# UWRobotLearning/WheeledLab

Measured on AMD Instinct MI355X. Metric: env steps/sec (whole node), drift task @ 4096 envs/GPU, higher is better.
Workload: dtype f32; 1 GPU; drift task, 4096 envs/GPU, flat terrain, fused step kernel, synthetic actions in HBM; envs_per_gpu=4096, total_envs=4096, parallelism=env-shard x1

## Files before the change

wheeledlab_amd/csrc/wl_drift.hip:

```cpp
#include "wl_drift_env.h"

namespace {

constexpr int kHotArgBytes = 56;

template <int LANES, class Ground, bool UNROLL = true, int DRIVE = -1, int QB = kBlock, bool STREAM = false>
__global__ void __launch_bounds__(kBlock, LANES == 4 ? WL_MIN_WAVES : (UNROLL ? WL_LANE_WAVES : WL_LOWREG_WAVES)) drift_step_kernel(float* __restrict__ state, int32_t* __restrict__ episode_len,
                                                            const float2* __restrict__ actions, const int stride,
                                                            const int n_envs, const int env_offset, const uint64_t seed,
                                                            const uint64_t step, const WlDriftParams p_arg,
                                                            const VehDerived vd_arg, const WlEnvBuffers b_arg,
                                                            const float* __restrict__ noise, const WlStepOut out,
                                                            const Ground ground, const MetricSlots slots) {
    constexpr int kEnvs = QB / LANES;
    WlDriftParams p = p_arg;
    VehDerived vd = vd_arg;
    WlEnvBuffers b = b_arg;
    b.state = state;
    b.episode_len = episode_len;
    b.stride = stride;
    b.n_envs = n_envs;
    b.env_offset = env_offset;
    __shared__ float tile[LANES == 1 ? kEnvs * kObsPad : 1];
    __shared__ float wave_metrics[LANES == 1 ? (QB / 64) * WL_M_COUNT : 1];
// ... 12 lines not shown
        float dr_mass, dr_mu_s, dr_mu_d, dr_damp;
        dr_mass = S.ld(WL_S_MASS, e), dr_mu_s = S.ld(WL_S_MU_S, e), dr_mu_d = S.ld(WL_S_MU_D, e), dr_damp = S.ld(WL_S_DAMP, e);
        load_rows<LANES>(S, b, p, e, wid, r);
        const uint32_t gid = (uint32_t)(b.env_offset + e);
        float* tile_w = tile + (LANES == 1 ? wave * 64 * kObsPad : 0);
        if constexpr (LANES == 4) {
            uint32_t kw[(sizeof(WlDriftParams) + sizeof(VehDerived)) / 4];
            kernarg_vector_words(kHotArgBytes, kw);
            int go = 1;
            asm volatile("" : "+s"(go) : : "memory");
            if (go) {
                StepDraws pre = draw_step_raw(gid, step, seed, wid);
                kernarg_words_landed(kw);
                __builtin_memcpy(&p, kw, sizeof(WlDriftParams));
                __builtin_memcpy(&vd, kw + sizeof(WlDriftParams) / 4, sizeof(VehDerived));
                keep_scalar_fields(p, p_arg);
                vd.n_sub = uniform_i32(vd.n_sub);
                ref_pose_request(pre, b.ref_poses, p.num_ref_points);
                env_const_rows(ec, p.vehicle, vd, dr_mass, dr_mu_s, dr_mu_d, dr_damp);
                drift_env_step<LANES>(p, b, vd, ground, S, ec, r, a, noise, out, e, wid, lead, gid, seed, step, tile_w, ms, nullptr, &pre);
            }
        } else {
            env_const_rows(ec, p.vehicle, vd, dr_mass, dr_mu_s, dr_mu_d, dr_damp);
            drift_env_step<LANES, UNROLL, DRIVE>(p, b, vd, ground, S, ec, r, a, noise, out, e, wid, lead, gid, seed, step, tile_w, ms);
        }
        store_rows<LANES>(S, b, p, e, wid, lead, r);
    }
    if (b.metrics_slots > 1) clear_metric_slot(b, slots.next);
    if constexpr (LANES == 1) {
        const int wave_env0 = blockIdx.x * kEnvs + wave * 64;
        if (wave_env0 < b.n_envs) flush_obs_wave<kStreaming>(tile + wave * 64 * kObsPad, out.obs, wave_env0, b.n_envs);
        ms.close();
    }
}

template <class Ground, int QB = kBlock >
__global__ void __launch_bounds__(kBlock) drift_rollout_kernel(const WlDriftParams p_arg, const WlEnvBuffers b,
                                                               const float2* __restrict__ actions, const WlStepOut out,
                                                               const int64_t obs_step_stride, const int64_t vec_step_stride,
                                                               const int n_steps, const uint64_t seed, const uint64_t step0,
                                                               const Ground ground, const VehDerived vd_arg, const MetricSlots slots) {
    constexpr int LANES = 4, kEnvs = QB / LANES;
    WlDriftParams p = p_arg;
    VehDerived vd = vd_arg;
    pin_params_vgpr(p, vd);
    const int wid = threadIdx.x & 3;
    const bool lead = wid == 0;
    const int e = blockIdx.x * kEnvs + threadIdx.x / LANES;
    if (b.metrics_slots > 1) clear_metric_slot(b, slots.next);
    if (e >= b.n_envs) return;
    const MetricSink<LANES> ms{nullptr, metric_shard(b, slots.cur)};
    const Rows S = make_rows(b.state, b.stride);
    EnvConst ec;
    DriftRows r;
    load_env_const(S, p.vehicle, vd, e, ec);
    load_rows<LANES>(S, b, p, e, wid, r);
    const uint32_t gid = (uint32_t)(b.env_offset + e);
    float2 a_next = n_steps > 0 ? actions[e] : make_float2(0.f, 0.f);
    for (int k = 0; k < n_steps; ++k) {
        WlStepOut o = out;
        o.obs += k * obs_step_stride;
        o.reward += k * vec_step_stride;
        o.terminated += k * vec_step_stride;
        o.truncated += k * vec_step_stride;
        if (o.dones) o.dones += k * vec_step_stride;
        const float2 a = a_next;
        if (k + 1 < n_steps) a_next = actions[(int64_t)(k + 1) * b.n_envs + e];
        const StepDraws pre = draw_step(p, b.ref_poses, gid, step0 + (uint64_t)k, seed, wid);
        drift_env_step<LANES>(p, b, vd, ground, S, ec, r, a, nullptr, o, e, wid, lead, gid, seed, step0 + (uint64_t)k, nullptr, ms,
                              nullptr, &pre);
    }
    store_rows<LANES>(S, b, p, e, wid, lead, r);
}

constexpr int kSplitEnvs = 16;
constexpr int kSplitBlock = 128;
constexpr int kSnapVec = 6, kDrawVec = 3;

WL_DEV void snap_publish(float4* slot, int q, const DriftSnap& s) {
    float4* w = slot + q * kSnapVec;
    w[0] = make_float4(s.pos.x, s.pos.y, s.pos.z, s.q.w);
    w[1] = make_float4(s.q.x, s.q.y, s.q.z, s.v.x);
    w[2] = make_float4(s.v.y, s.v.z, s.wb.x, s.wb.y);
    w[3] = make_float4(s.wb.z, s.wwz, s.th, s.a0);
    w[4] = make_float4(s.a1, __int_as_float(s.ep_len), __int_as_float(s.flags), s.dvx);
    w[5] = make_float4(s.dvy, s.dwz_hf, s.dwz_lf, 0.f);
}
WL_DEV DriftSnap snap_read(const float4* slot, int q) {
    const float4* w = slot + q * kSnapVec;
    const float4 w0 = w[0], w1 = w[1], w2 = w[2], w3 = w[3], w4 = w[4], w5 = w[5];
    DriftSnap s;
    s.pos = v3(w0.x, w0.y, w0.z), s.q = Quat{w0.w, w1.x, w1.y, w1.z}, s.v = v3(w1.w, w2.x, w2.y), s.wb = v3(w2.z, w2.w, w3.x);
    s.wwz = w3.y, s.th = w3.z, s.a0 = w3.w, s.a1 = w4.x, s.ep_len = __float_as_int(w4.y), s.flags = __float_as_int(w4.z);
    s.dvx = w4.w, s.dvy = w5.x, s.dwz_hf = w5.y, s.dwz_lf = w5.z;
    return s;
}
WL_DEV void draws_publish(float4* slot, int q, const DriftEventDraws& d) {
    float4* w = slot + q * kDrawVec;
    w[0] = make_float4(d.rx, d.ry, d.rqw, d.rqz);
    w[1] = make_float4(d.rt_hf, d.rt_lf, d.lf_kick, d.lf_timer);
    w[2] = make_float4(d.hf.x, d.hf.y, d.hf.z, d.hf.w);
}
WL_DEV DriftEventDraws draws_read(const float4* slot, int q) {
    const float4* w = slot + q * kDrawVec;
    const float4 w0 = w[0], w1 = w[1], w2 = w[2];
    DriftEventDraws d;
    d.rx = w0.x, d.ry = w0.y, d.rqw = w0.z, d.rqz = w0.w, d.rt_hf = w1.x, d.rt_lf = w1.y, d.lf_kick = w1.z, d.lf_timer = w1.w;
    d.hf = F4{w2.x, w2.y, w2.z, w2.w};
    return d;
}

template <class Ground>
__global__ void __launch_bounds__(kSplitBlock) drift_rollout_split_kernel(const WlDriftParams p_arg, const WlEnvBuffers b,
                                                                          const float2* __restrict__ actions, const WlStepOut out,
                                                                          const int64_t obs_step_stride, const int64_t vec_step_stride,
                                                                          const int n_steps, const uint64_t seed, const uint64_t step0,
                                                                          const Ground ground, const VehDerived vd_arg, const MetricSlots slots) {
    __shared__ float4 snap[2][kSplitEnvs * kSnapVec];
    __shared__ float4 drw[2][kSplitEnvs * kDrawVec];
    WlDriftParams p = p_arg;
    VehDerived vd = vd_arg;
    const int role = __builtin_amdgcn_readfirstlane((int)threadIdx.x >> 6);
    const int wid = threadIdx.x & 3, q = (threadIdx.x & 63) >> 2;
    const int e_quad = blockIdx.x * kSplitEnvs + q;
    if (b.metrics_slots > 1) clear_metric_slot(b, slots.next);
    if (blockIdx.x * kSplitEnvs >= b.n_envs) return;
    const bool live = e_quad < b.n_envs;
    const int e = live ? e_quad : b.n_envs - 1;
    const bool lead = wid == 0;
    const Rows S = make_rows(b.state, b.stride);
    const uint32_t gid = (uint32_t)(b.env_offset + e);
    if (role == 0) {
        pin_state_params_vgpr(p, vd);
        EnvConst ec;
        DriftRows r;
        load_env_const(S, p.vehicle, vd, e, ec);
        load_rows<4>(S, b, p, e, wid, r);
        float2 a_next = n_steps > 0 ? actions[e] : make_float2(0.f, 0.f);
        __syncthreads();
        for (int k = 0; k < n_steps; ++k) {
            const float2 a = a_next;
            if (k + 1 < n_steps) a_next = actions[(int64_t)(k + 1) * b.n_envs + e];
            const DriftEventDraws dr = draws_read(drw[k & 1], q);
            const DriftSnap sn = drift_state_half(p, vd, ground, ec, r, a, wid, dr);
            if (lead) snap_publish(snap[k & 1], q, sn);
            __syncthreads();
        }
        if (live) {
            WlDriftParams ps = p;
            ps.log_episode_sums = 0;
            store_rows<4>(S, b, ps, e, wid, lead, r);
        }
    } else {
        pin_output_params_vgpr(p);
        const MetricSink<4> ms{nullptr, metric_shard(b, slots.cur)};
        float epsum[WL_DR_NTERMS];
#pragma unroll
        for (int i = 0; i < WL_DR_NTERMS; ++i) epsum[i] = S.ld(WL_S_EPSUM0 + i, e);
        StepDraws d = draw_step(p, b.ref_poses, gid, step0, seed, wid);
        ResetDraw rd = quad_reset_draw(p, d);
        const DriftEventDraws ev0 = event_draws(rd, d);
        if (lead) draws_publish(drw[0], q, ev0);
        __syncthreads();
        for (int k = 0; k < n_steps; ++k) {
            WlStepOut o = out;
            o.obs += k * obs_step_stride;
            o.reward += k * vec_step_stride;
            o.terminated += k * vec_step_stride;
            o.truncated += k * vec_step_stride;
            if (o.dones) o.dones += k * vec_step_stride;
            const StepDraws dn = draw_step(p, b.ref_poses, gid, step0 + (uint64_t)(k + 1), seed, wid);
            const ResetDraw rdn = quad_reset_draw(p, dn);
            const DriftEventDraws evn = event_draws(rdn, dn);
            if (lead) draws_publish(drw[(k + 1) & 1], q, evn);
            __syncthreads();
            const DriftSnap sn = snap_read(snap[k & 1], q);
            drift_output_half(p, o, sn, rd, d.z, epsum, e, wid, live, ms);
            d = dn;
            rd = rdn;
        }
        if (live && lead && p.log_episode_sums) {
#pragma unroll
            for (int i = 0; i < WL_DR_NTERMS; ++i) S.st(WL_S_EPSUM0 + i, e, epsum[i]);
        }
    }
}

__global__ void __launch_bounds__(kBlock) drift_mdp_kernel(const WlDriftParams p, int n, int64_t stride,
                                                           const float* __restrict__ pos, const float* __restrict__ quat,
                                                           const float* __restrict__ vb_, const float* __restrict__ wb_,
                                                           const float* __restrict__ ww_, const float* __restrict__ steer,
                                                           const float* __restrict__ act, const uint8_t* __restrict__ timed_out,
                                                           float* __restrict__ terms, float* __restrict__ reward,
                                                           uint8_t* __restrict__ terminated, float* __restrict__ obs) {
    __shared__ float tile[kBlock * kObsPad];
    const int e = blockIdx.x * kBlock + threadIdx.x;
    if (e < n) {
        const V3 P = v3(pos[e], pos[stride + e], pos[2 * stride + e]);
        const Quat q{quat[e], quat[stride + e], quat[2 * stride + e], quat[3 * stride + e]};
        const V3 vb = v3(vb_[e], vb_[stride + e], vb_[2 * stride + e]);
        const V3 wb = v3(wb_[e], wb_[stride + e], wb_[2 * stride + e]);
        const float wwz = ww_[2 * stride + e];
        const float sm = 0.5f * (steer[e] + steer[stride + e]);
        const bool to = timed_out ? timed_out[e] != 0 : false;
        const bool term = cart_off_track(P.x, P.y, p.straight, p.r_in, p.r_out);
        const DriftTerms tm = drift_terms(p, P, vb, wb, wwz, sm, term, to, atan2_fast(vb.y, vb.x));
        const float step_dt = p.sim_dt * (float)p.decimation;
        float r = 0.f;
#pragma unroll
        for (int i = 0; i < WL_DR_NTERMS; ++i) {
            terms[i * stride + e] = tm.t[i];
            if (p.weight[i] != 0.f) r += tm.t[i] * p.weight[i] * step_dt;
        }
        reward[e] = r;
        terminated[e] = term ? 1 : 0;
        Noise12 zero;
#pragma unroll
        for (int k = 0; k < 12; ++k) zero.z[k] = 0.f;
        write_obs_row(&tile[threadIdx.x * kObsPad], p, P, euler_xyz_from_quat(q), vb, wb, act[e], act[stride + e], zero);
    }
    __syncthreads();
    flush_obs(tile, obs, blockIdx.x * kBlock, n);
}

__global__ void __launch_bounds__(kBlock) action_map_kernel(const WlActionParams ap, int n, const float2* __restrict__ actions,
                                                            float2* __restrict__ processed, float2* __restrict__ steer_target,
                                                            float4* __restrict__ wheel_target) {
    const int e = blockIdx.x * kBlock + threadIdx.x;
    if (e >= n) return;
    float2 a = actions[e];
    float v, delta, st, w[4];
    process_action(ap, a.x, a.y, v, delta);
    joint_targets(ap, v, delta, st, w);
    float sl, sr;
    steer_pair(ap, delta, st, sl, sr);
    processed[e] = make_float2(v, delta);
    steer_target[e] = make_float2(sl, sr);
    wheel_target[e] = make_float4(w[0], w[1], w[2], w[3]);
}

__global__ void __launch_bounds__(kBlock) drift_reset_kernel(const WlDriftParams p, const WlEnvBuffers b,
                                                             const uint8_t* __restrict__ mask, uint64_t seed, uint64_t step) {
    const int e = blockIdx.x * kBlock + threadIdx.x;
    if (e >= b.n_envs) return;
    if (mask && !mask[e]) return;
    const Rows S = make_rows(b.state, b.stride);
    const ResetDraw rd = draw_reset(p, b.ref_poses, (uint32_t)(b.env_offset + e), step, seed);
    store_reset_rows(S, b, e, rd.pos, rd.q, v3(0.f, 0.f, 0.f));
    S.st(WL_S_TIMER_HF, e, rd.timer_hf);
    S.st(WL_S_TIMER_LF, e, rd.timer_lf);
}

__global__ void __launch_bounds__(kBlock) drift_observe_kernel(const WlDriftParams p, const WlEnvBuffers b,
                                                               const float* __restrict__ noise, float* __restrict__ obs,
                                                               uint64_t seed, uint64_t step) {
    __shared__ float tile[kBlock * kObsPad];
    const int e = blockIdx.x * kBlock + threadIdx.x;
    if (e < b.n_envs) {
        const Rows S = make_rows(b.state, b.stride);
        const Quat q{S.ld(WL_S_QW, e), S.ld(WL_S_QX, e), S.ld(WL_S_QY, e), S.ld(WL_S_QZ, e)};
        const Mat3 R = mat_from_quat(q);
        const V3 vb = mul_t(R, ld3(S, WL_S_VX, e)), wb = mul_t(R, ld3(S, WL_S_WX, e));
// ... 202 lines not shown
```

wheeledlab_amd/csrc/wl_drift_env.h:

```cpp
#pragma once
#include <hip/hip_runtime.h>

#include "../../include/wheeledlab_amd.h"
#include "wl_kernel_common.h"
#include "wl_drift_terms.h"
#include "wl_rng.h"
#include "wl_vehicle.h"

namespace {

#ifndef WL_MIN_WAVES
#define WL_MIN_WAVES 2
#endif
constexpr int kObsDim = 14;
constexpr int kObsPad = 15;

struct ResetDraw {
    V3 pos;
    Quat q;
    float yaw;
    float timer_hf, timer_lf;
};

WL_DEV ResetDraw reset_from_uniforms(const WlDriftParams& p, const float* __restrict__ ref, F4 u , float t_hf, float t_lf) {
// ... 389 lines not shown
    bool hf_due = false;
    if (p.enable_pushes) {
        timer_hf -= step_dt;
        hf_due = timer_hf < 1e-6f;
    }
    U4 nb = U4{0u, 0u, 0u, 0u};
    const bool draw_noise = p.enable_corruption && !noise;
    if constexpr (LANES == 1) {
        if (draw_noise || hf_due) nb = philox_block(gid, step, WL_RS_NOISE1, seed);
    }
    if (p.enable_pushes) {
        if (hf_due) {
            F4 u;
            if constexpr (LANES == 4) u = quad_hf_draw(*pre);
            else u = u16x4(nb.z, nb.w);
            const float dvx = (2.f * u.x - 1.f) * p.hf_vel_x, dvy = (2.f * u.y - 1.f) * p.hf_vel_y, dwz = (2.f * u.z - 1.f) * p.hf_vel_yaw;
            s.v.x += dvx;
            s.v.y += dvy;
            ww.z += dwz;
            vb = v3(fmaf(Ro.r0.x, dvx, fmaf(Ro.r1.x, dvy, vb.x)), fmaf(Ro.r0.y, dvx, fmaf(Ro.r1.y, dvy, vb.y)),
                    fmaf(Ro.r0.z, dvx, fmaf(Ro.r1.z, dvy, vb.z)));
            wb_o = fma3(dwz, Ro.r2, wb_o);
            timer_hf = fmaf(u.w, p.hf_interval[1] - p.hf_interval[0], p.hf_interval[0]);
        }
        timer_lf = done ? timer_lf - step_dt : lf_next;
        if (timer_lf < 1e-6f) {
            float uk, ut;
            if constexpr (LANES == 4) quad_lf_draw(*pre, uk, ut);
            else uk = u16_lo(ev.w), ut = u16_hi(ev.w);
            const float dwz = (2.f * uk - 1.f) * p.lf_vel_yaw;
            ww.z += dwz;
            wb_o = fma3(dwz, Ro.r2, wb_o);
            timer_lf = fmaf(ut, p.lf_interval[1] - p.lf_interval[0], p.lf_interval[0]);
        }
    }
    r.pos = pos;
    r.q = s.q;
    r.v = s.v;
    r.ww = ww;
#pragma unroll
    for (int i = 0; i < 4; ++i) r.wheel[i] = s.wheel[i];
    r.th = s.th;
    r.om = s.om;
    r.a0 = a0;
    r.a1 = a1;
    r.timer_hf = timer_hf;
    r.timer_lf = timer_lf;
    r.ep_len = ep_len;
    if constexpr (LANES == 4) {
#pragma unroll
        for (int i = 0; i < WL_DR_NTERMS; ++i) r.epsum[i] = epsum[i];
    } else {
        if (p.log_episode_sums) {
#pragma unroll
            for (int i = 0; i < WL_DR_NTERMS; ++i) S.st(WL_S_EPSUM0 + i, e, epsum[i]);
        }
    }
    const V3 wb2 = wb_o;
    Noise12 nz;
    bool drawn = false;
    if constexpr (LANES == 4) {
        if (p.enable_corruption && !noise) {
            nz = gather_quad_noise(pre->z);
            drawn = true;
        }
    }
    if (!drawn) nz = obs_noise<LANES>(p, noise, b.stride, e, gid, step, seed, LANES == 1 ? &nb : nullptr);
    if constexpr (LANES == 1) euler = euler_xyz_from_quat(s.q);
    if constexpr (LANES == 4) {
        float o_local[14];
        float* o = obs_keep ? obs_keep : o_local;
        obs_values(o, p, pos, euler, vb, wb2, a0, a1, nz);
        if (!obs_keep) store_obs_quad(out.obs + (int64_t)e * kObsDim, wid, o);
    } else {
        write_obs_row(&tile[(threadIdx.x & 63) * kObsPad], p, pos, euler, vb, wb2, a0, a1, nz);
    }
}

struct DriftSnap {
    V3 pos;
    Quat q;
    V3 v, wb;
    float wwz, th;
    float a0, a1;
    int ep_len;
    int flags;
    float dvx, dvy, dwz_hf, dwz_lf;
};
enum { kSnapFinite = 1, kSnapTerminated = 2, kSnapTruncated = 4, kSnapHf = 8, kSnapLf = 16 };
struct DriftEventDraws {
    float rx, ry, rqw, rqz, rt_hf, rt_lf;
    float lf_kick, lf_timer;
    F4 hf;
};
WL_DEV DriftEventDraws event_draws(const ResetDraw& rd, const StepDraws& d) {
    DriftEventDraws ev;
    ev.rx = rd.pos.x, ev.ry = rd.pos.y, ev.rqw = rd.q.w, ev.rqz = rd.q.z, ev.rt_hf = rd.timer_hf, ev.rt_lf = rd.timer_lf;
    quad_lf_draw(d, ev.lf_kick, ev.lf_timer);
    ev.hf = quad_hf_draw(d);
    return ev;
}

template <class Ground>
WL_DEV DriftSnap drift_state_half(const WlDriftParams& p, const VehDerived& vd, const Ground& ground, EnvConst& ec, DriftRows& r,
                                  float2 a, int wid, const DriftEventDraws& dr) {
    const WlVehicleParams& vp = p.vehicle;
    float v_t, delta;
    process_action(p.action, a.x, a.y, v_t, delta);
    joint_targets(p.action, v_t, delta, ec.steer_target, ec.wheel_target);
    env_const_lane(ec, vp, vd, wid);
    VehState s;
    s.q = r.q;
    s.v = r.v;
#pragma unroll
    for (int i = 0; i < 4; ++i) s.wheel[i] = r.wheel[i];
    s.th = r.th;
    s.om = r.om;
    {
        const Mat3 R = mat_from_quat(s.q);
        s.x = r.pos + vp.cg_z * v3(R.r0.z, R.r1.z, R.r2.z);
        s.wb = mul_t(R, r.ww);
    }
    vehicle_integrate<4, Ground, true, -1>(vp, vd, ec, s, ground, wid);
    const Mat3 R = mat_from_quat(s.q);
    V3 ww = mul(R, s.wb);
    V3 pos = s.x - vp.cg_z * v3(R.r0.z, R.r1.z, R.r2.z);
    const float wheel_sum = quad_sum(s.wheel[0]);
    const float chk_in[16] = {pos.x, pos.y, pos.z, s.q.w, s.q.x, s.q.y, s.q.z, s.v.x, s.v.y, s.v.z, ww.x, ww.y, ww.z, wheel_sum, s.th, s.om};
    const bool finite = __builtin_isfinite(sum16(chk_in));
    const bool terminated = !finite || cart_off_track(pos.x, pos.y, p.straight, p.r_in, p.r_out);
    int ep_len = r.ep_len + 1;
    const bool truncated = ep_len >= p.max_episode_length;
    const float step_dt = p.sim_dt * (float)p.decimation;
    DriftSnap sn;
    sn.pos = pos, sn.q = s.q, sn.v = s.v, sn.wb = s.wb, sn.wwz = ww.z, sn.th = s.th, sn.a0 = a.x, sn.a1 = a.y, sn.ep_len = ep_len;
    sn.flags = (finite ? kSnapFinite : 0) | (terminated ? kSnapTerminated : 0) | (truncated ? kSnapTruncated : 0);
    sn.dvx = sn.dvy = sn.dwz_hf = sn.dwz_lf = 0.f;
    float a0 = a.x, a1 = a.y, timer_hf = r.timer_hf, timer_lf = r.timer_lf;
    const float lf_next = timer_lf - step_dt;
    const bool done = terminated || truncated;
    if (done) {
        if (!finite) {
#pragma unroll
            for (int i = 0; i < 4; ++i) s.wheel[i] = 0.f;
            s.th = s.om = 0.f;
        }
        pos = v3(dr.rx, dr.ry, 0.f);
        s.q = Quat{dr.rqw, 0.f, 0.f, dr.rqz};
        s.v = v3(0.f, 0.f, 0.f);
        ww = v3(0.f, 0.f, 0.f);
        timer_hf = dr.rt_hf;
        timer_lf = dr.rt_lf;
        ep_len = 0;
        a0 = a1 = 0.f;
    }
    bool hf_due = false;
    if (p.enable_pushes) {
        timer_hf -= step_dt;
        hf_due = timer_hf < 1e-6f;
        if (hf_due) {
            const F4 u = dr.hf;
            const float dvx = (2.f * u.x - 1.f) * p.hf_vel_x, dvy = (2.f * u.y - 1.f) * p.hf_vel_y, dwz = (2.f * u.z - 1.f) * p.hf_vel_yaw;
            s.v.x += dvx;
            s.v.y += dvy;
            ww.z += dwz;
            sn.dvx = dvx, sn.dvy = dvy, sn.dwz_hf = dwz;
            sn.flags |= kSnapHf;
            timer_hf = fmaf(u.w, p.hf_interval[1] - p.hf_interval[0], p.hf_interval[0]);
        }
        timer_lf = done ? timer_lf - step_dt : lf_next;
        if (timer_lf < 1e-6f) {
            const float dwz = (2.f * dr.lf_kick - 1.f) * p.lf_vel_yaw;
            ww.z += dwz;
            sn.dwz_lf = dwz;
            sn.flags |= kSnapLf;
            timer_lf = fmaf(dr.lf_timer, p.lf_interval[1] - p.lf_interval[0], p.lf_interval[0]);
        }
    }
    r.pos = pos;
    r.q = s.q;
    r.v = s.v;
    r.ww = ww;
#pragma unroll
    for (int i = 0; i < 4; ++i) r.wheel[i] = s.wheel[i];
    r.th = s.th;
    r.om = s.om;
    r.a0 = a0;
    r.a1 = a1;
    r.timer_hf = timer_hf;
    r.timer_lf = timer_lf;
    r.ep_len = ep_len;
    return sn;
}

WL_DEV void drift_output_half(const WlDriftParams& p, const WlStepOut& out, const DriftSnap& sn, const ResetDraw& rd, const float z[4],
                              float epsum_rows[WL_DR_NTERMS], int e, int wid, bool live, const MetricSink<4>& ms) {
    const bool lead = wid == 0 && live;
    const bool finite = sn.flags & kSnapFinite, terminated = sn.flags & kSnapTerminated, truncated = sn.flags & kSnapTruncated;
    float epsum[WL_DR_NTERMS];
#pragma unroll
    for (int i = 0; i < WL_DR_NTERMS; ++i) epsum[i] = p.log_episode_sums ? epsum_rows[i] : 0.f;
    V3 pos = sn.pos;
    const Mat3 R = mat_from_quat(sn.q);
    V3 vb = mul_t(R, sn.v);
    float slip_angle;
    V3 euler;
    {
        const Quat q = sn.q;
        const float sp = 2.f * fmaf(q.w, q.y, -(q.z * q.x));
        const float ay = quad_pick(wid, opaque(vb.y), opaque(2.f * fmaf(q.y, q.z, q.w * q.x)), opaque(sp), opaque(2.f * fmaf(q.x, q.y, q.w * q.z)));
        const float ax = quad_pick(wid, opaque(vb.x), opaque(fmaf(fmaf(q.x, q.x, q.y * q.y), -2.f, 1.f)), opaque(fsqrt(fmaxf(fmaf(-sp, sp, 1.f), 0.f))),
                                   opaque(fmaf(fmaf(q.z, q.z, q.y * q.y), -2.f, 1.f)));
        const float ang = atan2_fast(ay, ax);
        slip_angle = quad_bcast<0>(ang);
        euler = v3(wrap_2pi(quad_bcast<1>(ang)), wrap_2pi(quad_bcast<2>(ang)), wrap_2pi(quad_bcast<3>(ang)));
    }
    const int ep_len = sn.ep_len;
    DriftTerms tm = drift_terms(p, pos, vb, sn.wb, sn.wwz, sn.th, terminated, truncated, slip_angle);
    const float step_dt = p.sim_dt * (float)p.decimation;
    float reward = 0.f;
#pragma unroll
    for (int i = 0; i < WL_DR_NTERMS; ++i) {
        const float w = p.weight[i];
        const float c = (w != 0.f && finite) ? tm.t[i] * w * step_dt : 0.f;
        reward += c;
        epsum[i] += c;
    }
    if (lead) {
        out.reward[e] = reward;
        out.terminated[e] = terminated ? 1 : 0;
        out.truncated[e] = truncated ? 1 : 0;
        if (out.dones) out.dones[e] = (terminated || truncated) ? 1 : 0;
    }
    Mat3 Ro = R;
    V3 wb_o = sn.wb;
    float a0 = sn.a0, a1 = sn.a1;
    const bool done = terminated || truncated;
    if (done) {
        if (lead) {
#pragma unroll
            for (int i = 0; i < WL_DR_NTERMS; ++i) ms.add(WL_M_EPSUM0 + i, epsum[i]);
            ms.add(WL_M_RESETS, 1.f);
            if (truncated) ms.add(WL_M_TIMEOUTS, 1.f);
            if (terminated) ms.add(WL_M_TERM0, 1.f);
            if (!finite) ms.add(WL_M_NONFINITE, 1.f);
            ms.add(WL_M_EPLEN, (float)ep_len);
        }
#pragma unroll
        for (int i = 0; i < WL_DR_NTERMS; ++i) epsum[i] = 0.f;
        pos = rd.pos;
        euler = v3(0.f, 0.f, rd.yaw - WL_TWO_PI * floorf(rd.yaw * WL_INV_TWO_PI));
        vb = v3(0.f, 0.f, 0.f);
        wb_o = v3(0.f, 0.f, 0.f);
        const float cy = fmaf(rd.q.w, rd.q.w, -rd.q.z * rd.q.z), sy = 2.f * rd.q.w * rd.q.z;
        Ro = Mat3{v3(cy, -sy, 0.f), v3(sy, cy, 0.f), v3(0.f, 0.f, 1.f)};
        a0 = a1 = 0.f;
    }
    if (sn.flags & kSnapHf) {
        const float dvx = sn.dvx, dvy = sn.dvy, dwz = sn.dwz_hf;
        vb = v3(fmaf(Ro.r0.x, dvx, fmaf(Ro.r1.x, dvy, vb.x)), fmaf(Ro.r0.y, dvx, fmaf(Ro.r1.y, dvy, vb.y)),
                fmaf(Ro.r0.z, dvx, fmaf(Ro.r1.z, dvy, vb.z)));
        wb_o = fma3(dwz, Ro.r2, wb_o);
    }
    if (sn.flags & kSnapLf) wb_o = fma3(sn.dwz_lf, Ro.r2, wb_o);
#pragma unroll
    for (int i = 0; i < WL_DR_NTERMS; ++i) epsum_rows[i] = epsum[i];
    Noise12 nz;
    if (p.enable_corruption) {
        nz = gather_quad_noise(z);
    } else {
#pragma unroll
        for (int k = 0; k < 12; ++k) nz.z[k] = 0.f;
    }
    float o[14];
    obs_values(o, p, pos, euler, vb, wb_o, a0, a1, nz);
    if (live) store_obs_quad(out.obs + (int64_t)e * kObsDim, wid, o);
}

WL_DEV void pin_vgpr(float& x) { asm volatile("" : "+v"(x)); }
template <int N>
WL_DEV void pin_vgpr(float (&a)[N]) {
#pragma unroll
    for (int i = 0; i < N; ++i) pin_vgpr(a[i]);
}
WL_DEV void pin_params_vgpr(WlDriftParams& p, VehDerived& d) {
    pin_vgpr(p.sim_dt);
    WlActionParams& a = p.action;
    pin_vgpr(a.scale), pin_vgpr(a.offset), pin_vgpr(a.base_length), pin_vgpr(a.base_width), pin_vgpr(a.wheel_radius);
    WlVehicleParams& v = p.vehicle;
    float* vf[] = {&v.gravity, &v.half_wheelbase_f, &v.half_wheelbase_r, &v.half_track, &v.wheel_radius, &v.wheel_z, &v.cg_z,
                   &v.gyr_x, &v.gyr_y, &v.gyr_z, &v.wheel_inertia, &v.wheel_damping, &v.susp_k, &v.susp_c, &v.ground_mu_s,
                   &v.ground_mu_d, &v.slip_peak, &v.v_min, &v.motor_sat, &v.motor_limit, &v.motor_vel_limit, &v.steer_kp,
                   &v.steer_kd, &v.steer_effort, &v.steer_vel_limit, &v.steer_inertia, &v.susp_fmax};
#pragma unroll
    for (float* f : vf) pin_vgpr(*f);
    float* pf[] = {&p.straight, &p.r_in, &p.r_out, &p.r_line, &p.slip_min, &p.slip_max, &p.slip_min_vx, &p.speed_target,
                   &p.speed_offset, &p.tlgr_thresh, &p.ctd_offset, &p.ctd_p, &p.pos_noise, &p.yaw_noise, &p.hf_vel_x,
                   &p.hf_vel_y, &p.hf_vel_yaw, &p.lf_vel_yaw};
#pragma unroll
    for (float* f : pf) pin_vgpr(*f);
    pin_vgpr(p.weight), pin_vgpr(p.noise_std), pin_vgpr(p.hf_interval), pin_vgpr(p.lf_interval);
    float* df[] = {&d.h, &d.inv_h, &d.half_h, &d.steer_a, &d.steer_b, &d.steer_J_h, &d.steer_h_J, &d.zrel, &d.Iw_h, &d.A0,
                   &d.inv_wlim, &d.mot_b, &d.r2, &d.inv_A0, &d.hg, &d.inv_g2x, &d.inv_g2y, &d.inv_g2z, &d.cgx, &d.cgy, &d.cgz};
#pragma unroll
    for (float* f : df) pin_vgpr(*f);
}

WL_DEV void pin_state_params_vgpr(WlDriftParams& p, VehDerived& d) {
    pin_vgpr(p.sim_dt);
    WlActionParams& a = p.action;
    pin_vgpr(a.scale), pin_vgpr(a.offset), pin_vgpr(a.base_length), pin_vgpr(a.base_width), pin_vgpr(a.wheel_radius);
    WlVehicleParams& v = p.vehicle;
    float* vf[] = {&v.gravity, &v.half_wheelbase_f, &v.half_wheelbase_r, &v.half_track, &v.wheel_radius, &v.wheel_z, &v.cg_z,
                   &v.gyr_x, &v.gyr_y, &v.gyr_z, &v.wheel_inertia, &v.wheel_damping, &v.susp_k, &v.susp_c, &v.ground_mu_s,
                   &v.ground_mu_d, &v.slip_peak, &v.v_min, &v.motor_sat, &v.motor_limit, &v.motor_vel_limit, &v.steer_kp,
                   &v.steer_kd, &v.steer_effort, &v.steer_vel_limit, &v.steer_inertia, &v.susp_fmax};
#pragma unroll
    for (float* f : vf) pin_vgpr(*f);
    float* pf[] = {&p.straight, &p.r_in, &p.r_out, &p.hf_vel_x, &p.hf_vel_y, &p.hf_vel_yaw, &p.lf_vel_yaw};
#pragma unroll
    for (float* f : pf) pin_vgpr(*f);
    pin_vgpr(p.hf_interval), pin_vgpr(p.lf_interval);
    float* df[] = {&d.h, &d.inv_h, &d.half_h, &d.steer_a, &d.steer_b, &d.steer_J_h, &d.steer_h_J, &d.zrel, &d.Iw_h, &d.A0,
                   &d.inv_wlim, &d.mot_b, &d.r2, &d.inv_A0, &d.hg, &d.inv_g2x, &d.inv_g2y, &d.inv_g2z, &d.cgx, &d.cgy, &d.cgz};
#pragma unroll
    for (float* f : df) pin_vgpr(*f);
}
WL_DEV void pin_output_params_vgpr(WlDriftParams& p) {
    pin_vgpr(p.sim_dt);
    float* pf[] = {&p.straight, &p.r_line, &p.slip_min, &p.slip_max, &p.slip_min_vx, &p.speed_target, &p.speed_offset,
                   &p.tlgr_thresh, &p.ctd_offset, &p.ctd_p, &p.pos_noise, &p.yaw_noise};
#pragma unroll
    for (float* f : pf) pin_vgpr(*f);
    pin_vgpr(p.weight), pin_vgpr(p.noise_std), pin_vgpr(p.hf_interval), pin_vgpr(p.lf_interval);
}

WL_DEV void keep_scalar_fields(WlDriftParams& v, const WlDriftParams&) {
    uniform_scalar_common(v);
    v.enable_corruption = uniform_i32(v.enable_corruption);
    v.num_ref_points = uniform_i32(v.num_ref_points);
    v.enable_pushes = uniform_i32(v.enable_pushes);
}

inline int check_buffers(const WlDriftParams* p, const WlEnvBuffers* b) {
    if (!p || !b || !b->state || !b->episode_len || !b->ref_poses || !b->metrics) return WL_EINVAL;
    if (b->n_envs <= 0 || b->stride < b->n_envs) return WL_EINVAL;
    if (b->stride % 64 != 0 || ((uintptr_t)b->state & 15u)) return WL_EALIGN;
    if (b->metrics_slots < 1 || (b->lanes != 0 && b->lanes != 1 && b->lanes != 2 && b->lanes != 4)) return WL_EINVAL;
    if (!flags_ok(b) || ((b->flags & WL_FLAG_STREAM) && b->lanes == 4)) return WL_EINVAL;
    if (b->stride * 4 * WL_S_COUNT > 0x7fffffffLL) return WL_EINVAL;
    if (p->decimation <= 0 || p->vehicle.substeps <= 0 || p->num_ref_points <= 0 || p->num_ref_points > 32) return WL_EINVAL;
    if (p->vehicle.implicit != 0 || !(p->vehicle.susp_fmax > 0.f)) return WL_EINVAL;
    if (!(p->sim_dt > 0.f)) return WL_EINVAL;
    return WL_OK;
}

}
```

wheeledlab_amd/csrc/wl_vehicle.h:

```cpp
#pragma once
#include "../../include/wheeledlab_amd.h"
#include "wl_math.h"

struct VehState {
    V3 x;
    Quat q;
    V3 v;
    V3 wb;
    float wheel[4];
    float th, om;
};

struct EnvConst {
    float h_inv_mass;
    float K_cap;
    float mu_s, mu_d, mu_sd;
    float damp;
    float inv_A0_damp;
    float steer_target;
    float wheel_target[4];
    float wt_lane, bx_lane, by_lane, d_lane, inv_A0d_lane;
    float lx_lane, ly_lane;
};

// ... 7 lines not shown
    float hg;
    float inv_g2x, inv_g2y, inv_g2z;
    float cgx, cgy, cgz;
    float inv_wlim, mot_b;
    float mot_g;
    float r2;
    float Dn;
    float az2, bx2, by2;
    float gz, inv_gz;
    float lxf, lxr, ly;
    float iso_x, iso_y, iso_z;
    int32_t n_sub;
};

inline VehDerived derive_vehicle(const WlVehicleParams& vp, float sim_dt, int decimation) {
    VehDerived d;
    d.h = sim_dt / (float)vp.substeps;
    d.inv_h = 1.f / d.h;
    d.half_h = 0.5f * d.h;
    const float invJ = 1.f / vp.steer_inertia;
    d.steer_a = d.h * vp.steer_kp * invJ;
    d.steer_b = 1.f / (1.f + d.h * vp.steer_kd * invJ + d.h * d.h * vp.steer_kp * invJ);
    d.steer_J_h = vp.steer_inertia * d.inv_h;
    d.steer_h_J = d.h * invJ;
    d.zrel = vp.wheel_z - vp.cg_z;
    d.Iw_h = vp.wheel_inertia * d.inv_h;
    d.A0 = d.Iw_h + vp.wheel_damping;
    d.inv_A0 = 1.f / d.A0;
    d.hg = d.h * vp.gravity;
    const float gx2 = vp.gyr_x * vp.gyr_x, gy2 = vp.gyr_y * vp.gyr_y, gz2 = vp.gyr_z * vp.gyr_z;
    d.inv_g2x = 1.f / gx2;
    d.inv_g2y = 1.f / gy2;
    d.inv_g2z = 1.f / gz2;
    d.cgx = d.h * (gz2 - gy2) / gx2;
    d.cgy = d.h * (gx2 - gz2) / gy2;
    d.cgz = d.h * (gy2 - gx2) / gz2;
    d.inv_wlim = 1.f / vp.motor_vel_limit;
    d.mot_b = vp.motor_sat / vp.motor_vel_limit;
    d.mot_g = 10.f / vp.motor_limit;
    d.r2 = vp.wheel_radius * vp.wheel_radius;
    d.Dn = vp.susp_c + d.h * vp.susp_k;
    const float az = d.zrel - vp.wheel_radius;
    d.az2 = az * az;
    d.bx2 = 0.5f * (vp.half_wheelbase_f * vp.half_wheelbase_f + vp.half_wheelbase_r * vp.half_wheelbase_r);
    d.by2 = vp.half_track * vp.half_track;
    d.gz = vp.gyr_z;
    d.inv_gz = 1.f / vp.gyr_z;
    d.lxf = vp.half_wheelbase_f * d.inv_gz;
    d.lxr = -vp.half_wheelbase_r * d.inv_gz;
    d.ly = vp.half_track * d.inv_gz;
    const float rho2 = d.bx2 + d.by2 + d.az2;
    d.iso_x = rho2 * d.inv_g2x, d.iso_y = rho2 * d.inv_g2y, d.iso_z = rho2 * d.inv_g2z;
    d.n_sub = decimation * vp.substeps;
    return d;
}

WL_DEV void env_const_rows(EnvConst& ec, const WlVehicleParams& vp, const VehDerived& vd, float mass, float mu_s_wheel,
                           float mu_d_wheel, float damp) {
    ec.h_inv_mass = vd.h * rcp(mass);
    ec.K_cap = 0.125f * mass * vd.inv_h;
    ec.mu_s = mu_s_wheel * vp.ground_mu_s;
    ec.mu_d = fminf(mu_d_wheel * vp.ground_mu_d, ec.mu_s);
    ec.mu_sd = ec.mu_s - ec.mu_d;
    ec.damp = damp;
    ec.inv_A0_damp = rcp(vd.A0 + damp);
}

struct FlatGround {
    static constexpr bool kFlat = true;
    WL_DEV void sample(float, float, float& zg, V3& n) const {
        zg = 0.f;
        n = v3(0.f, 0.f, 1.f);
    }
    template <int W>
    WL_DEV void sample_wheel(float x, float y, float& zg, V3& n) const { sample(x, y, zg, n); }
};

WL_DEV float quad_pick(int wid, float a, float b, float c, float d) { return wid == 0 ? a : wid == 1 ? b : wid == 2 ? c : d; }

WL_DEV void env_const_lane(EnvConst& ec, const WlVehicleParams& vp, const VehDerived& vd, int wid) {
    const bool front = wid >= 2, left = (wid & 1) == 0;
    const bool driven = (vp.drive == 1) || !front;
    ec.wt_lane = quad_pick(wid, ec.wheel_target[0], ec.wheel_target[1], ec.wheel_target[2], ec.wheel_target[3]);
    ec.bx_lane = front ? vp.half_wheelbase_f : -vp.half_wheelbase_r;
    ec.by_lane = left ? vp.half_track : -vp.half_track;
    ec.d_lane = driven ? ec.damp : 0.f;
    ec.inv_A0d_lane = driven ? ec.inv_A0_damp : vd.inv_A0;
    ec.lx_lane = front ? vd.lxf : vd.lxr;
    ec.ly_lane = left ? vd.ly : -vd.ly;
}

struct TyreCoef {
    float fx, fy, kz;
    float Fz;
    float kx, ky;
    float dk;
};
template <bool STEER>
WL_DEV V3 tyre_force(float fx, float fy, float kz, V3 n, float hc, float hs) {
    const float fyz = fy * n.z;
    if constexpr (STEER) return v3(fmaf(kz, n.x, fmaf(fx, hc, -fyz * hs)), fmaf(kz, n.y, fmaf(fx, hs, fyz * hc)),
                                   fmaf(kz, n.z, fy * fmaf(n.x, hs, -n.y * hc)));
    else return v3(fmaf(kz, n.x, fx), fmaf(kz, n.y, fyz), fmaf(kz, n.z, -fy * n.y));
}
template <bool STEER, bool MOTOR, bool IMPL = false>
WL_DEV TyreCoef wheel_tyre(const WlVehicleParams& vp, const VehDerived& vd, const EnvConst& ec, V3 n, V3 vc, float pen, float hc,
                           float hs, float d, float inv_A0d, float wt, float& w_spin) {
    const float r = vp.wheel_radius;
    const float vn = dot(n, vc);
    const float Fz = pen > 0.f ? fmaxf(fmaf(-vp.susp_c, vn, fminf(vp.susp_k * pen, vp.susp_fmax)), 0.f) : 0.f;
    const float g = STEER ? fmaf(n.x, hc, n.y * hs) : n.x;
    const float m = STEER ? fmaf(n.x, hs, -n.y * hc) : -n.y;
    const float lx = STEER ? fmaf(hc, vc.x, hs * vc.y) : vc.x;
    const float ly = STEER ? fmaf(hc, vc.y, -hs * vc.x) : vc.y;
    const float it = rsq(fmaxf(fmaf(-g, g, 1.f), 1e-6f));
    const float vcx = it * fmaf(-g, vn, lx);
    const float vcy = it * fmaf(n.z, ly, m * vc.z);
    const float w_i = w_spin;
    const float wr = w_i * r;
    const float vden = fmaxf(vp.v_min, vp.slip_peak * fmaxf(fabsf(vcx), fabsf(wr)));
    const float inv_vden = rcp(vden);
    const float sx = (wr - vcx) * inv_vden, sy = vcy * inv_vden;
    const float s2 = fmaxf(fmaf(sx, sx, sy * sy), 1e-30f);
    const float rs = rsq(s2);
    const float sig = s2 * rs;
    const float inv_sig = fminf(rs, 1.f);
    const float gq = fmaf(ec.mu_s, fmaxf(1.f - sig, 0.f), fmaf(ec.mu_sd, inv_sig, ec.mu_d) * inv_sig);
    const float K = IMPL ? Fz * gq * inv_vden : fminf(Fz * gq * inv_vden, ec.K_cap);
    const float A = fmaf(K, vd.r2, vd.A0);
    const float rK = r * K;
    const float rhs0 = fmaf(vd.Iw_h, w_i, rK * vcx);
    const float inv_A = rcp(A);
    float w_n, tau_lo = 0.f, tau_hi = 0.f;
    float cw = inv_A;
    if constexpr (MOTOR) {
        tau_hi = clampf(fmaf(-vd.mot_b, w_i, vp.motor_sat), 0.f, vp.motor_limit);
        tau_lo = clampf(fmaf(-vd.mot_b, w_i, -vp.motor_sat), -vp.motor_limit, 0.f);
        const float inv_Ad = rcp(A + d);
        const float w_u = fmaf(d, wt, rhs0) * inv_Ad;
        w_n = clampf(w_u, (rhs0 + tau_lo) * inv_A, (rhs0 + tau_hi) * inv_A);
        if constexpr (IMPL) {
            const float m_hi = fmaf(-A, w_u, rhs0 + tau_hi), m_lo = fmaf(A, w_u, -(rhs0 + tau_lo));
            cw = fmaf(clampf(fminf(m_hi, m_lo) * vd.mot_g, 0.f, 1.f), inv_Ad - inv_A, inv_A);
        }
    } else {
        w_n = rhs0 * inv_A;
    }
    float ks = K;
    float Fx = fmaf(w_n, rK, -K * vcx);
    float Fy = -K * vcy;
    const float Fmax = ec.mu_s * Fz;
    const float mag2 = fmaf(Fx, Fx, Fy * Fy);
    if (mag2 > Fmax * Fmax) {
        const float scale = Fmax * rsq(fmaxf(mag2, 1e-30f));
        Fx *= scale;
        Fy *= scale;
        if constexpr (IMPL) ks = K * scale;
        const float rhs2 = fmaf(vd.Iw_h, w_i, -r * Fx);
        if constexpr (MOTOR) {
            const float w_u2 = fmaf(d, wt, rhs2) * inv_A0d;
            w_n = clampf(w_u2, (rhs2 + tau_lo) * vd.inv_A0, (rhs2 + tau_hi) * vd.inv_A0);
        } else {
            w_n = rhs2 * vd.inv_A0;
        }
    }
    w_spin = w_n;
// ... 274 lines not shown
```

Baseline: 1.392 billion env-steps/s.

## Move action processing into output wave and pass targets via shared memory

```diff
diff --git a/wheeledlab_amd/csrc/wl_drift.hip b/wheeledlab_amd/csrc/wl_drift.hip
--- a/wheeledlab_amd/csrc/wl_drift.hip
+++ b/wheeledlab_amd/csrc/wl_drift.hip
@@ -118,17 +118,17 @@
     w[0] = make_float4(s.pos.x, s.pos.y, s.pos.z, s.q.w);
     w[1] = make_float4(s.q.x, s.q.y, s.q.z, s.v.x);
     w[2] = make_float4(s.v.y, s.v.z, s.wb.x, s.wb.y);
-    w[3] = make_float4(s.wb.z, s.wwz, s.th, s.a0);
-    w[4] = make_float4(s.a1, __int_as_float(s.ep_len), __int_as_float(s.flags), s.dvx);
-    w[5] = make_float4(s.dvy, s.dwz_hf, s.dwz_lf, 0.f);
+    w[3] = make_float4(s.wb.z, s.wwz, s.th, __int_as_float(s.ep_len));
+    w[4] = make_float4(__int_as_float(s.flags), s.dvx, s.dvy, s.dwz_hf);
+    w[5].x = s.dwz_lf;
 }
 WL_DEV DriftSnap snap_read(const float4* slot, int q) {
     const float4* w = slot + q * kSnapVec;
-    const float4 w0 = w[0], w1 = w[1], w2 = w[2], w3 = w[3], w4 = w[4], w5 = w[5];
+    const float4 w0 = w[0], w1 = w[1], w2 = w[2], w3 = w[3], w4 = w[4];
     DriftSnap s;
     s.pos = v3(w0.x, w0.y, w0.z), s.q = Quat{w0.w, w1.x, w1.y, w1.z}, s.v = v3(w1.w, w2.x, w2.y), s.wb = v3(w2.z, w2.w, w3.x);
-    s.wwz = w3.y, s.th = w3.z, s.a0 = w3.w, s.a1 = w4.x, s.ep_len = __float_as_int(w4.y), s.flags = __float_as_int(w4.z);
-    s.dvx = w4.w, s.dvy = w5.x, s.dwz_hf = w5.y, s.dwz_lf = w5.z;
+    s.wwz = w3.y, s.th = w3.z, s.ep_len = __float_as_int(w3.w), s.flags = __float_as_int(w4.x);
+    s.dvx = w4.y, s.dvy = w4.z, s.dwz_hf = w4.w, s.dwz_lf = w[5].x;
     return s;
 }
 WL_DEV void draws_publish(float4* slot, int q, const DriftEventDraws& d) {
@@ -144,6 +144,13 @@
     d.rx = w0.x, d.ry = w0.y, d.rqw = w0.z, d.rqz = w0.w, d.rt_hf = w1.x, d.rt_lf = w1.y, d.lf_kick = w1.z, d.lf_timer = w1.w;
     d.hf = F4{w2.x, w2.y, w2.z, w2.w};
     return d;
+}
+WL_DEV void action_publish(float4* slot, int lane, const DriftActionRec& r) {
+    slot[lane] = make_float4(r.steer_target, r.wt_lane, r.a0, r.a1);
+}
+WL_DEV DriftActionRec action_read(const float4* slot, int lane) {
+    const float4 w = slot[lane];
+    return DriftActionRec{w.x, w.y, w.z, w.w};
 }
 
 template <class Ground>
@@ -154,10 +161,11 @@
                                                                           const Ground ground, const VehDerived vd_arg, const MetricSlots slots) {
     __shared__ float4 snap[2][kSplitEnvs * kSnapVec];
     __shared__ float4 drw[2][kSplitEnvs * kDrawVec];
+    __shared__ float4 act[2][64];
     WlDriftParams p = p_arg;
     VehDerived vd = vd_arg;
     const int role = __builtin_amdgcn_readfirstlane((int)threadIdx.x >> 6);
-    const int wid = threadIdx.x & 3, q = (threadIdx.x & 63) >> 2;
+    const int lane = threadIdx.x & 63, wid = lane & 3, q = lane >> 2;
     const int e_quad = blockIdx.x * kSplitEnvs + q;
     if (b.metrics_slots > 1) clear_metric_slot(b, slots.next);
     if (blockIdx.x * kSplitEnvs >= b.n_envs) return;
@@ -171,14 +179,13 @@
         EnvConst ec;
         DriftRows r;
         load_env_const(S, p.vehicle, vd, e, ec);
+        ec.mu_sd = fmaf(S.ld(WL_S_MU_S, e), p.vehicle.ground_mu_s, -ec.mu_d);
         load_rows<4>(S, b, p, e, wid, r);
-        float2 a_next = n_steps > 0 ? actions[e] : make_float2(0.f, 0.f);
         __syncthreads();
         for (int k = 0; k < n_steps; ++k) {
-            const float2 a = a_next;
-            if (k + 1 < n_steps) a_next = actions[(int64_t)(k + 1) * b.n_envs + e];
+            const DriftActionRec ar = action_read(act[k & 1], lane);
             const DriftEventDraws dr = draws_read(drw[k & 1], q);
-            const DriftSnap sn = drift_state_half(p, vd, ground, ec, r, a, wid, dr);
+            const DriftSnap sn = drift_state_half(p, vd, ground, ec, r, ar, wid, dr);
             if (lead) snap_publish(snap[k & 1], q, sn);
             __syncthreads();
         }
@@ -197,6 +204,12 @@
         ResetDraw rd = quad_reset_draw(p, d);
         const DriftEventDraws ev0 = event_draws(rd, d);
         if (lead) draws_publish(drw[0], q, ev0);
+        float2 a_first = make_float2(0.f, 0.f), a_next = make_float2(0.f, 0.f);
+        if (n_steps > 0) a_first = actions[e];
+        if (n_steps > 1) a_next = actions[(int64_t)b.n_envs + e];
+        DriftActionRec ac = drift_action_ahead(p.action, a_first, wid);
+        action_publish(act[0], lane, ac);
+        const ActionSwitches asw = park_action_switches(p.action);
         __syncthreads();
         for (int k = 0; k < n_steps; ++k) {
             WlStepOut o = out;
@@ -209,11 +222,15 @@
             const ResetDraw rdn = quad_reset_draw(p, dn);
             const DriftEventDraws evn = event_draws(rdn, dn);
             if (lead) draws_publish(drw[(k + 1) & 1], q, evn);
+            const DriftActionRec an = drift_action_ahead(with_action_switches(p.action, asw), a_next, wid);
+            if (k + 2 < n_steps) a_next = actions[(int64_t)(k + 2) * b.n_envs + e];
+            action_publish(act[(k + 1) & 1], lane, an);
             __syncthreads();
             const DriftSnap sn = snap_read(snap[k & 1], q);
-            drift_output_half(p, o, sn, rd, d.z, epsum, e, wid, live, ms);
+            drift_output_half(p, o, sn, rd, d.z, epsum, ac.a0, ac.a1, e, wid, live, ms);
             d = dn;
             rd = rdn;
+            ac = an;
         }
         if (live && lead && p.log_episode_sums) {
 #pragma unroll
diff --git a/wheeledlab_amd/csrc/wl_drift_env.h b/wheeledlab_amd/csrc/wl_drift_env.h
--- a/wheeledlab_amd/csrc/wl_drift_env.h
+++ b/wheeledlab_amd/csrc/wl_drift_env.h
@@ -495,7 +495,6 @@
     Quat q;
     V3 v, wb;
     float wwz, th;
-    float a0, a1;
     int ep_len;
     int flags;
     float dvx, dvy, dwz_hf, dwz_lf;
@@ -514,14 +513,44 @@
     return ev;
 }
 
+struct DriftActionRec {
+    float steer_target, wt_lane;
+    float a0, a1;
+};
+WL_DEV DriftActionRec drift_action_ahead(const WlActionParams& ap, float2 a, int wid) {
+    DriftActionRec rec;
+    float v, delta;
+    process_action(ap, a.x, a.y, v, delta);
+    rec.a0 = a.x, rec.a1 = a.y;
+    const float t = tan_fast(delta);
+    rec.steer_target = ap.map == 2 ? delta : t;
+    const float inv_r = 1.f / ap.wheel_radius;
+    float w0, w1, w2, w3;
+    if (ap.map == 0) {
+        w0 = w1 = v * inv_r;
+        w2 = w3 = 0.f;
+    } else {
+        const float L = ap.base_length, W2 = 0.5f * ap.base_width;
+        const float R = (t == 0.f) ? 1e6f : L / t;
+        const float inv_Rr = 1.f / (R * ap.wheel_radius);
+        const float dl = R - W2, dr = R + W2, LL = L * L;
+        const float rl = sqrtf(fmaf(dl, dl, LL)), rr = sqrtf(fmaf(dr, dr, LL));
+        w0 = v * fabsf(dl * inv_Rr);
+        w1 = v * fabsf(dr * inv_Rr);
+        w2 = v * fabsf(rl * inv_Rr);
+        w3 = v * fabsf(rr * inv_Rr);
+    }
+    rec.wt_lane = quad_pick(wid, w0, w1, w2, w3);
+    return rec;
+}
+
 template <class Ground>
 WL_DEV DriftSnap drift_state_half(const WlDriftParams& p, const VehDerived& vd, const Ground& ground, EnvConst& ec, DriftRows& r,
-                                  float2 a, int wid, const DriftEventDraws& dr) {
+                                  const DriftActionRec& act, int wid, const DriftEventDraws& dr) {
     const WlVehicleParams& vp = p.vehicle;
-    float v_t, delta;
-    process_action(p.action, a.x, a.y, v_t, delta);
-    joint_targets(p.action, v_t, delta, ec.steer_target, ec.wheel_target);
-    env_const_lane(ec, vp, vd, wid);
+    ec.steer_target = act.steer_target;
+    ec.wt_lane = act.wt_lane;
+    env_const_lane_fixed(ec, vp, vd, wid);
     VehState s;
     s.q = r.q;
     s.v = r.v;
@@ -546,10 +575,10 @@
     const bool truncated = ep_len >= p.max_episode_length;
     const float step_dt = p.sim_dt * (float)p.decimation;
     DriftSnap sn;
-    sn.pos = pos, sn.q = s.q, sn.v = s.v, sn.wb = s.wb, sn.wwz = ww.z, sn.th = s.th, sn.a0 = a.x, sn.a1 = a.y, sn.ep_len = ep_len;
+    sn.pos = pos, sn.q = s.q, sn.v = s.v, sn.wb = s.wb, sn.wwz = ww.z, sn.th = s.th, sn.ep_len = ep_len;
     sn.flags = (finite ? kSnapFinite : 0) | (terminated ? kSnapTerminated : 0) | (truncated ? kSnapTruncated : 0);
     sn.dvx = sn.dvy = sn.dwz_hf = sn.dwz_lf = 0.f;
-    float a0 = a.x, a1 = a.y, timer_hf = r.timer_hf, timer_lf = r.timer_lf;
+    float a0 = act.a0, a1 = act.a1, timer_hf = r.timer_hf, timer_lf = r.timer_lf;
     const float lf_next = timer_lf - step_dt;
     const bool done = terminated || truncated;
     if (done) {
@@ -607,7 +636,8 @@
 }
 
 WL_DEV void drift_output_half(const WlDriftParams& p, const WlStepOut& out, const DriftSnap& sn, const ResetDraw& rd, const float z[4],
-                              float epsum_rows[WL_DR_NTERMS], int e, int wid, bool live, const MetricSink<4>& ms) {
+                              float epsum_rows[WL_DR_NTERMS], float act_a0, float act_a1, int e, int wid, bool live,
+                              const MetricSink<4>& ms) {
     const bool lead = wid == 0 && live;
     const bool finite = sn.flags & kSnapFinite, terminated = sn.flags & kSnapTerminated, truncated = sn.flags & kSnapTruncated;
     float epsum[WL_DR_NTERMS];
@@ -647,7 +677,7 @@
     }
     Mat3 Ro = R;
     V3 wb_o = sn.wb;
-    float a0 = sn.a0, a1 = sn.a1;
+    float a0 = act_a0, a1 = act_a1;
     const bool done = terminated || truncated;
     if (done) {
         if (lead) {
@@ -721,8 +751,6 @@
 
 WL_DEV void pin_state_params_vgpr(WlDriftParams& p, VehDerived& d) {
     pin_vgpr(p.sim_dt);
-    WlActionParams& a = p.action;
-    pin_vgpr(a.scale), pin_vgpr(a.offset), pin_vgpr(a.base_length), pin_vgpr(a.base_width), pin_vgpr(a.wheel_radius);
     WlVehicleParams& v = p.vehicle;
     float* vf[] = {&v.gravity, &v.half_wheelbase_f, &v.half_wheelbase_r, &v.half_track, &v.wheel_radius, &v.wheel_z, &v.cg_z,
                    &v.gyr_x, &v.gyr_y, &v.gyr_z, &v.wheel_inertia, &v.wheel_damping, &v.susp_k, &v.susp_c, &v.ground_mu_s,
@@ -741,11 +769,28 @@
 }
 WL_DEV void pin_output_params_vgpr(WlDriftParams& p) {
     pin_vgpr(p.sim_dt);
+    WlActionParams& a = p.action;
+    pin_vgpr(a.scale), pin_vgpr(a.offset), pin_vgpr(a.base_length), pin_vgpr(a.base_width), pin_vgpr(a.wheel_radius);
     float* pf[] = {&p.straight, &p.r_line, &p.slip_min, &p.slip_max, &p.slip_min_vx, &p.speed_target, &p.speed_offset,
                    &p.tlgr_thresh, &p.ctd_offset, &p.ctd_p, &p.pos_noise, &p.yaw_noise};
 #pragma unroll
     for (float* f : pf) pin_vgpr(*f);
     pin_vgpr(p.weight), pin_vgpr(p.noise_std), pin_vgpr(p.hf_interval), pin_vgpr(p.lf_interval);
+}
+
+struct ActionSwitches {
+    int clip_wrapper, bounding, map, no_reverse;
+};
+WL_DEV ActionSwitches park_action_switches(const WlActionParams& ap) {
+    ActionSwitches s{ap.clip_wrapper, ap.bounding, ap.map, ap.no_reverse};
+    asm volatile("" : "+v"(s.clip_wrapper), "+v"(s.bounding), "+v"(s.map), "+v"(s.no_reverse));
+    return s;
+}
+WL_DEV WlActionParams with_action_switches(WlActionParams ap, ActionSwitches s) {
+    asm volatile("" : "+v"(s.clip_wrapper), "+v"(s.bounding), "+v"(s.map), "+v"(s.no_reverse));
+    ap.clip_wrapper = __builtin_amdgcn_readfirstlane(s.clip_wrapper), ap.bounding = __builtin_amdgcn_readfirstlane(s.bounding);
+    ap.map = __builtin_amdgcn_readfirstlane(s.map), ap.no_reverse = __builtin_amdgcn_readfirstlane(s.no_reverse);
+    return ap;
 }
 
 WL_DEV void keep_scalar_fields(WlDriftParams& v, const WlDriftParams&) {
diff --git a/wheeledlab_amd/csrc/wl_vehicle.h b/wheeledlab_amd/csrc/wl_vehicle.h
--- a/wheeledlab_amd/csrc/wl_vehicle.h
+++ b/wheeledlab_amd/csrc/wl_vehicle.h
@@ -113,6 +113,16 @@
     const bool front = wid >= 2, left = (wid & 1) == 0;
     const bool driven = (vp.drive == 1) || !front;
     ec.wt_lane = quad_pick(wid, ec.wheel_target[0], ec.wheel_target[1], ec.wheel_target[2], ec.wheel_target[3]);
+    ec.bx_lane = front ? vp.half_wheelbase_f : -vp.half_wheelbase_r;
+    ec.by_lane = left ? vp.half_track : -vp.half_track;
+    ec.d_lane = driven ? ec.damp : 0.f;
+    ec.inv_A0d_lane = driven ? ec.inv_A0_damp : vd.inv_A0;
+    ec.lx_lane = front ? vd.lxf : vd.lxr;
+    ec.ly_lane = left ? vd.ly : -vd.ly;
+}
+WL_DEV void env_const_lane_fixed(EnvConst& ec, const WlVehicleParams& vp, const VehDerived& vd, int wid) {
+    const bool front = wid >= 2, left = (wid & 1) == 0;
+    const bool driven = (vp.drive == 1) || !front;
     ec.bx_lane = front ? vp.half_wheelbase_f : -vp.half_wheelbase_r;
     ec.by_lane = left ? vp.half_track : -vp.half_track;
     ec.d_lane = driven ? ec.damp : 0.f;
```

After: 1.451 billion env-steps/s, median of 6. 4.2% higher.
